# yukara-ikemiya/world-class

Measured on AMD Instinct MI355X. Metric: analysis+synthesis frames/sec (whole node), 48 kHz 5 ms hop, higher is better.
Workload: dtype f64; 1 GPU; 64 synthetic 48 kHz 10 s utterances per GPU (8 distinct, tiled), 5 ms hop, Harvest->CheapTrick->D4C->Synthesis, inputs resident in HBM when the clock starts (`value`; SURVEY.md section 8(d)'s headline with H2D of x and D2H of all outputs inside the clock is `value_with_transfers`); utterances_per_gpu=64, frames_per_gpu=128064, fs=48000, fft_size=2048, parallelism=utterance-sharded x1 (shard.partition), final RCCL all-gather of F0 + checksums

## Files before the change

### world_class_amd/build.py

```python
import hashlib
import os
import re
import subprocess
import sys
from concurrent.futures import ThreadPoolExecutor

HERE = os.path.dirname(os.path.abspath(__file__))
CSRC = os.path.join(HERE, "csrc")
OUT = os.path.join(HERE, "libworldclass_hip.so")
OBJ = os.path.join(HERE, "_obj")
EXTRA = os.environ.get("WC_EXTRA_FLAGS", "").split()
FLAGS = EXTRA + ["--offload-arch=gfx950", "-O3", "-std=c++17", "-fPIC", "-ffp-contract=off", "-munsafe-fp-atomics", "-Wall",
         "-Wno-unused-function", "-Wno-unused-result", "-mllvm", "-simplifycfg-sink-common=false"]
HASH_MARKER = b"WC_SOURCE_HASH="


def sources():
    return sorted(f for f in os.listdir(CSRC) if f.endswith(".hip"))


def headers():
    inc = os.path.join(os.path.dirname(HERE), "include")
    hs = sorted(os.path.join(CSRC, f) for f in os.listdir(CSRC) if f.endswith(".hpp"))
    hs += [os.path.join(inc, f) for f in ("world_class_c.h", "world_class_io.h", "world_class_codec.h", "world_class_stream.h", "world_class_shard.h",
                                          "world_matlabfunctions.hpp", "world_fft.hpp") if os.path.exists(os.path.join(inc, f))]
    return hs


def source_hash():
    h = hashlib.sha256()
    h.update(" ".join(FLAGS).encode())
    for path in [os.path.join(CSRC, f) for f in sources()] + headers():
        h.update(b"\0" + os.path.basename(path).encode() + b"\0")
        with open(path, "rb") as f:
            h.update(f.read())
    return h.hexdigest()


def embedded_hash(path=None):
    path = path or OUT
    if not os.path.exists(path):
        return None
    with open(path, "rb") as f:
        m = re.search(HASH_MARKER + rb"([0-9a-f]{64})", f.read())
    return m.group(1).decode() if m else None


def _stale(out, deps):
    if not os.path.exists(out):
        return True
    t = os.path.getmtime(out)
    return any(os.path.getmtime(d) > t for d in deps)


def build(force=False, verbose=False):
    hipcc = os.environ.get("HIPCC", "/opt/rocm/bin/hipcc")
    want = source_hash()
    if not force and embedded_hash() == want:
        return OUT
    os.makedirs(OBJ, exist_ok=True)
    stamp = os.path.join(OBJ, "flags.txt")
    flags_now = " ".join(FLAGS)
    if not os.path.exists(stamp) or open(stamp).read() != flags_now:
        force = True
    jobs = []
    objs = []
    hs = headers()
    for src in sources():
        s = os.path.join(CSRC, src)
        o = os.path.join(OBJ, src[:-4] + ".o")
        objs.append(o)
        cmd = [hipcc] + FLAGS
        if src == "wc_core.hip":
            cmd += ['-DWC_SOURCE_HASH="%s"' % want]
            jobs.append(cmd + ["-c", s, "-o", o])
        elif force or _stale(o, [s] + hs):
            jobs.append(cmd + ["-c", s, "-o", o])

    def run(cmd):
        if verbose:
            print(" ".join(cmd), flush=True)
        r = subprocess.run(cmd, stdout=subprocess.PIPE, stderr=subprocess.STDOUT, text=True)
        return r.returncode, r.stdout

    with ThreadPoolExecutor(max_workers=4) as ex:
        for rc, out in ex.map(run, jobs):
            if out.strip():
                print(out)
            if rc != 0:
                raise RuntimeError("hipcc failed")
    with open(stamp, "w") as f:
        f.write(flags_now)
    rc, out = run([hipcc, "--offload-arch=gfx950", "-shared", "-fPIC", "-o", OUT] + objs + ["-ldl"])
    if out.strip():
        print(out)
    if rc != 0:
        raise RuntimeError("link failed")
    if embedded_hash() != want:
        raise RuntimeError("built library does not carry the expected source hash")
    return OUT


if __name__ == "__main__":
    print(build(force="--force" in sys.argv, verbose=True))
```

### world_class_amd/csrc/wc_stages.hpp

```cpp
#pragma once
#include <utility>
#include <vector>

#include "wc_internal.hpp"
#include "wc_stretch.hpp"

inline bool fft_size_supported(int fft_size) { return fft_size == 512 || fft_size == 1024 || fft_size == 2048 || fft_size == 4096; }

int hv_enqueue(wc_harvest *h, hipStream_t s, int n_utt, const double *d_x, const int *x_length, double *d_tpos, double *d_f0,
			   bool full, hipEvent_t mid_event, hipEvent_t start_after, int part = 3, hipEvent_t bp_done = nullptr,
			   hipEvent_t tail_after = nullptr);
int hv_overflowed(wc_harvest *h, hipStream_t s, bool *overflow, bool *tie = nullptr, std::vector<int> *tie_utts = nullptr);
std::vector<std::pair<int, int>> hv_runs_of(const std::vector<int> &us);
wc_harvest *hv_exact_twin(wc_harvest *h);
void hv_set_phases(wc_harvest *h, int mask);
int hv_row_width(const wc_harvest *h);
int hv_reserve_rows(wc_harvest *h, long long total_1ms_frames);
double *hv_candidate_rows(wc_harvest *h);
double *hv_score_rows(wc_harvest *h);

int ct_prepare(wc_cheaptrick *c, hipStream_t s, int n_utt, const int *x_length, const double *d_f0, const int *f0_length,
			   const uint64_t *rng_pos, long long *total_out, uint64_t *min_pos_out, uint64_t *max_end_out);
int ct_frames(wc_cheaptrick *c, hipStream_t s, int n_utt, const double *d_x, const double *d_tpos, const double *d_f0,
			  double *d_sp, long long total, hipEvent_t *rows_done);
const unsigned long long *ct_end_positions(const wc_cheaptrick *c);
void ct_set_f0_bound(wc_cheaptrick *c, double f0_bound);
void d4c_set_f0_bound(wc_d4c *d, double f0_bound);

int d4c_enqueue(wc_d4c *d, hipStream_t s, int n_utt, const double *d_x, const int *x_length, const double *d_tpos,
				const double *d_f0, const int *f0_length, int fft_size, double *d_ap, const uint64_t *rng_pos,
				const unsigned long long *d_start);
const unsigned long long *d4c_end_positions(const wc_d4c *d);
uint64_t d4c_draw_bound(const wc_d4c *d, int f0_length);

int syn_prepare(wc_synthesis *sy, hipStream_t s, int n_utt, const double *d_f0, const int *f0_length, const int *out_length,
				double *d_out, const uint64_t *rng_pos, bool full);
int syn_pulses(wc_synthesis *sy, hipStream_t s, const double *d_f0, const double *d_sp, const double *d_ap, double *d_out,
			   const unsigned long long *d_start);
int syn_finish(wc_synthesis *sy, hipStream_t s, uint64_t *rng_pos_out, bool *overflow);

wc::Device *hv_device(const wc_harvest *h);
wc::Device *ct_device(const wc_cheaptrick *c);
wc::Device *d4c_device(const wc_d4c *d);
wc::Device *syn_device(const wc_synthesis *sy);
const double *syn_dc_remover(const wc_synthesis *sy);
int syn_fs(const wc_synthesis *sy);

namespace wc {
struct CodecPlanArgs {
	const int *k;
	const double *s;
	const double2 *w;
};
struct CodecPlan {
	DevBuf k, s, w, kp, sp;
	CodecPlanArgs args() const { return {k.as<int>(), s.as<double>(), w.as<double2>()}; }
	CodecPlanArgs wave_args() const { return {kp.as<int>(), sp.as<double>(), w.as<double2>()}; }
};
int codec_plan(Device *dev, int fs, int fft_size, bool coding, const CodecPlan **out);
int codec_code_sp_launch(Device *dev, hipStream_t st, int fft_size, long long n_frames, int nd, const double *d_sp, double *d_coded,
						 const CodecPlan &pl);
int codec_decode_sp_launch(Device *dev, hipStream_t st, int fft_size, long long n_frames, int nd, const double *d_coded, double *d_sp,
						   const CodecPlan &pl);
int codec_code_ap_launch(hipStream_t st, int fs, int fft_size, long long n_frames, const double *d_ap, double *d_coded);
int codec_decode_ap_launch(hipStream_t st, int fs, int fft_size, long long n_frames, const double *d_coded, double *d_ap);

const char *decode_features_check(int fs, int fft_size, int nd);
int decode_features_enqueue(Device *dev, hipStream_t s, int fs, int fft_size, long long n_frames, int nd, const double *d_coded_sp,
							const double *d_coded_ap, const double *d_spectral_ratio, double *d_sp, double *d_ap);

int modify_frames_enqueue(hipStream_t s, int fs, int fft_size, long long n_frames, double *d_f0, double *d_sp, const double *d_f0_scale,
						  const double *d_spectral_ratio);

const char *retime_check(int fs, int fft_size, int n_utt, const int *in_length, const int *out_length, long long *total_out);
int retime_enqueue(Device *dev, hipStream_t s, int fs, int fft_size, int n_utt, const int *in_length, const double *d_f0_in,
				   const double *d_sp_in, const double *d_ap_in, const int *out_length, const double *d_position, const double *d_f0_scale,
				   const double *d_spectral_ratio, double *d_f0_out, double *d_sp_out, double *d_ap_out, long long total_out);

// ... 6 lines not shown
```

### world_class_amd/csrc/wc_synth_stream.hip

```cpp
#include <algorithm>
#include <cfloat>
#include <climits>
#include <cmath>
#include <cstring>
#include <vector>

#include "wc_stages.hpp"
#include "wc_synthesis.hpp"
#include "../../include/world_class_stream.h"

namespace wc {

struct SsDesc {
	long long win_old, win_new;
	long long in_off;
	int keep_from, keep, n_in;
	int f_base, f_len;
	int n0, n1;
	int cap;
	int has_pend, pend_idx, pend_vuv;
	double pend_shift;
	double run, wrap, vu;
	long long inc_off, slot;
};
// ... 480 lines not shown
		std::memcpy(h + ((char *)d_utt - dm), utt.data(), sizeof(UttDesc) * na);
		std::memcpy(h + ((char *)d_prefix - dm), prefix.data(), sizeof(long long) * (na + 1));
		std::memcpy(h + ((char *)d_capoff - dm), capoff.data(), sizeof(long long) * na);
		std::memcpy(h + ((char *)d_pairs - dm), pairs.data(), sizeof(long long) * 2 * na);
		std::memcpy(h + ((char *)d_first - dm), first.data(), sizeof(int) * na);
		const size_t off = (char *)d_ol - dm, len = ((char *)(d_first + na)) - (char *)d_ol;
		WC_HIP(hipMemcpyAsync(dm + off, h + off, len, hipMemcpyHostToDevice, hs));
		if ((rc = s->h_stage.mark(hs))) return rc;
	}
	double *carry_old = s->carry[par].as<double>(), *carry_new = s->carry[1 - par].as<double>();
	const unsigned tiles = (unsigned)std::max(1, (max_span + SS_TILE - 1) / SS_TILE);
	auto overlap = [&](const double *rows, const double *src, double *dst, const OlDesc *descs) {
		switch (N) {
			case 512: hipLaunchKernelGGL(ss_overlap_kernel<512>, dim3(tiles, na), dim3(SS_T), 0, hs, descs, (const int *)pb.index, rows, src, d_y, dst); break;
			case 1024: hipLaunchKernelGGL(ss_overlap_kernel<1024>, dim3(tiles, na), dim3(SS_T), 0, hs, descs, (const int *)pb.index, rows, src, d_y, dst); break;
			case 2048: hipLaunchKernelGGL(ss_overlap_kernel<2048>, dim3(tiles, na), dim3(SS_T), 0, hs, descs, (const int *)pb.index, rows, src, d_y, dst); break;
			default: hipLaunchKernelGGL(ss_overlap_kernel<4096>, dim3(tiles, na), dim3(SS_T), 0, hs, descs, (const int *)pb.index, rows, src, d_y, dst); break;
		}
	};
	std::vector<OlDesc> ol_expand;
	if (atomic) {
		if ((rc = s->work.reserve(sizeof(double) * (size_t)n * s->wsz))) return rc;
	}
	if (total_p > 0) {
		if (!atomic && (rc = s->resp.reserve(sizeof(double) * (size_t)total_p * N))) return rc;
		SynArgs sa;
		std::memset(&sa, 0, sizeof(sa));
		sa.utts = d_utt; sa.n_utt = na; sa.pulse_prefix = d_prefix; sa.cap_off = d_capoff; sa.first_index = d_first; sa.p = pb;
		sa.f0 = s->wf0[1 - par].as<double>(); sa.sp = s->wsp[1 - par].as<double>(); sa.ap = s->wap[1 - par].as<double>();
		sa.tw = s->dev->twiddle; sa.dc_remover = syn_dc_remover(s->sy);
		sa.out = atomic ? s->work.as<double>() : nullptr;
		sa.resp = atomic ? nullptr : s->resp.as<double>();
		sa.rng_start = nullptr; sa.trace = nullptr; sa.only_pulse = -1; sa.fs = s->fs; sa.frame_period = s->frame_period;
		std::vector<int> owner((size_t)total_p);
		for (int a = 0; a < na; ++a) std::fill(owner.begin() + prefix[a], owner.begin() + prefix[a + 1], a);
		DevBuf &pu = s->owner;
		if ((rc = pu.reserve(sizeof(int) * (size_t)total_p * 2))) return rc;
		WC_HIP(hipMemcpyAsync(pu.p, owner.data(), sizeof(int) * (size_t)total_p, hipMemcpyHostToDevice, hs));
		WC_HIP(hipMemsetAsync(pu.as<int>() + total_p, 0, sizeof(int) * (size_t)total_p, hs));
		WC_HIP(hipStreamSynchronize(hs));
		if (atomic) {
			std::vector<OlDesc> ex(ol);
			for (auto &d : ex) { d.dst_off = d.src_off / s->ccap * s->wsz; d.cut = d.lo; }
			ol_expand = ex;
		}
		uint64_t lo = ~0ull, hi = 0;
		for (int a = 0; a < na; ++a) {
			if (n_syn[a] == 0) continue;
			lo = std::min<uint64_t>(lo, start[a]);
			hi = std::max<uint64_t>(hi, start[a] + (uint64_t)(E[act[a]] - first[a]) + 1);
		}
		if (atomic) {
			if ((rc = s->aux.reserve(sizeof(OlDesc) * na))) return rc;
			WC_HIP(hipMemcpyAsync(s->aux.p, ol_expand.data(), sizeof(OlDesc) * na, hipMemcpyHostToDevice, hs));
			overlap(nullptr, carry_old, s->work.as<double>(), s->aux.as<OlDesc>());
			WC_HIP(hipStreamSynchronize(hs));
		}
		if (hi - lo <= (1ull << 28)) {
			if ((rc = s->dev->ensure_rng(lo, hi))) return rc;
			sa.rng_table = s->dev->rng_table.as<uint32_t>(); sa.rng_base = s->dev->rng_base;
			sa.pulse_utt = pu.as<int>();
			sa.total_pulses = total_p;
			if ((rc = syn_launch_responses(N, sa, hs))) return rc;
		} else {
			for (int a = 0; a < na; ++a) {
				if (n_syn[a] == 0) continue;
// ... 95 lines not shown
```

### world_class_amd/csrc/wc_synthesis.hip

```cpp
#include <cmath>
#include <cstdlib>
#include <cstring>
#include <vector>

#include "wc_device.hpp"
#include "wc_internal.hpp"
#include "wc_frames.hpp"
#include "wc_wavefft.hpp"
#include "wc_hostcopy.hpp"
#include "wc_synthesis.hpp"
#include "wc_stages.hpp"

namespace wc {

constexpr double kSafe = 0.000000000001;

struct TbArgs {
	const UttDesc *utts;
	const double *f0;
	const long long *cap_off;
	const int *cap;
	PulseBuf p;
	int *count;
	int *first_index;
// ... 1024 lines not shown
	wf_r2c_unpack(mr, mi, nyq, tw, lane);
#pragma unroll
	for (int s = 0; s < 16; ++s) {
		const double t = wf_exp_l(mr[s] * (0.5 / N), T);
		double sn, cs;
		wf_sincos(mi[s] * (0.5 / N), sn, cs);
		mr[s] = t * cs;
		mi[s] = t * sn;
	}
	mMr = wf_exp_l(nyq * (0.5 / N), T);
}

#ifndef WC_SYN_WAVE_OCC
#define WC_SYN_WAVE_OCC 2
#endif
#ifndef WC_SYN_ROWS_G
#define WC_SYN_ROWS_G 2
#endif
#ifndef WC_SYN_PARK_NOISE
#define WC_SYN_PARK_NOISE 1
#endif
#ifndef WC_SYN_ROW_PF
#define WC_SYN_ROW_PF 0
#endif
#ifndef WC_SYN_TRACE
#define WC_SYN_TRACE 0
#endif
#if WC_SYN_TRACE
#define SYN_STAMP(i) do { if (lane == 0) a.trace[gp * 16 + (i)] = __builtin_readcyclecounter(); } while (0)
#else
#define SYN_STAMP(i) do { } while (0)
#endif
template <bool ATOMIC>
__global__ __launch_bounds__(64) __attribute__((amdgpu_waves_per_eu(WC_SYN_WAVE_OCC, WC_SYN_WAVE_OCC))) void syn_pulse_wave_kernel(SynArgs a) {
	constexpr int N = 2048, M = 1024;
	__shared__ __attribute__((aligned(16))) double L[kWfLds];
	__shared__ __attribute__((aligned(16))) double T[kWfTabLds];
#if WC_SYN_PARK_NOISE
	__shared__ __attribute__((aligned(16))) double P[1024];
#endif
	const int lane = threadIdx.x;
#ifdef WC_SYN_LDS_PAD
	__shared__ double PAD[WC_SYN_LDS_PAD];
	if (a.fs < 0) PAD[lane] = 0.0;
#endif
	const long long total_p = a.pulse_prefix[a.n_utt];
	if ((long long)blockIdx.x >= 8 * ((total_p + 7) / 8)) return;
	const long long gp = xcd_frame(blockIdx.x, total_p);
	if (gp >= total_p) return;
	if (a.only_pulse >= 0 && gp != a.only_pulse) return;
	const int u = a.pulse_utt[gp];
	wf_tables_to_lds(T, a.tw, lane);
	const UttDesc ud = a.utts[u];
	const long long slot = a.cap_off[u] + (gp - a.pulse_prefix[u]);
	const int pidx = a.p.index[slot];
	const double shift = a.p.shift[slot];
	const int noise_size = a.p.noise_size[slot];
	const double vuv = (double)a.p.vuv[slot];
	const int fs = a.fs, Lf = ud.f_len;
	const double fp = a.frame_period;
	const double t = pidx / (double)fs;

	const int fl = min(Lf - 1, (int)floor(t / fp));
	const int ce = min(Lf - 1, (int)ceil(t / fp));
	const double ipol = uniform_d(t / fp - fl);
	const double *__restrict__ sf = a.sp + (ud.f_off + fl - ud.f_base) * (long long)(M + 1);
	const double *__restrict__ sc = a.sp + (ud.f_off + ce - ud.f_base) * (long long)(M + 1);
	const double *__restrict__ af = a.ap + (ud.f_off + fl - ud.f_base) * (long long)(M + 1);
	const double *__restrict__ ac = a.ap + (ud.f_off + ce - ud.f_base) * (long long)(M + 1);
	const bool same = fl == ce;
	auto blend = [&](double s0, double s1, double a0, double a1, double &env, double &ar) {
		if (same) {
			env = fabs(s0);
			const double s = safe_ap(a0);
			ar = s * s;
		} else {
			env = fma(1.0 - ipol, fabs(s0), ipol * fabs(s1));
			const double s = (1.0 - ipol) * safe_ap(a0) + ipol * safe_ap(a1);
			ar = s * s;
		}
	};
	double ar0;
	{
		double env;
		blend(sf[0], sc[0], af[0], ac[0], env, ar0);
		ar0 = uniform_d(ar0);
	}
#if WC_SYN_ROW_PF > 0
	double pf_s, pf_a;
	{
		const long long r2 = (ud.f_off + min(ce + WC_SYN_ROW_PF, Lf - 1) - ud.f_base) * (long long)(M + 1) + 16 * lane;
		pf_s = a.sp[r2];
		pf_a = a.ap[r2];
	}
#endif
	SYN_STAMP(0);
	SYN_STAMP(1);

	double dc = 0.0;
	const double sq = sqrt((double)noise_size);
#ifdef WC_SYN_RESP_ALIAS
	double *__restrict__ resp = a.resp + (gp & 2047) * (ATOMIC ? M : N);
#else
	double *__restrict__ resp = a.resp + gp * (ATOMIC ? M : N);
#endif
	double *__restrict__ yout = a.out + ud.y_off;
	const int ylen = ud.y_len;
	auto add2 = [&](int o, double v0, double v1) {
		if (o >= 0 && o < ylen) atomicAdd(yout + o, v0);
		if (o + 1 >= 0 && o + 1 < ylen) atomicAdd(yout + o + 1, v1);
	};
	const bool has_periodic = !(vuv <= 0.5 || ar0 > 0.999);
#pragma unroll 1
	for (int part = has_periodic ? 0 : 1; part < 2; ++part) {
		int ln = lane;
		WC_FRESH(ln);
		double wr[16], wi[16];
		double nr[16], ni[16], nsM = 0.0;
		if (part == 1) {
			const unsigned long long rstart = a.rng_start ? a.rng_start[u] : ud.rng_pos;
			const uint32_t *__restrict__ rng = a.rng_table + (rstart + (unsigned long long)(pidx - a.first_index[u]) - a.rng_base);
			double s = 0.0;
			{
				uint32_t raw[32];
#pragma unroll
				for (int q = 0; q < 16; ++q) {
					if ((q & 3) == 0 && q * 128 >= noise_size) break;
					const int i0 = 2 * ln + 128 * q;
					raw[2 * q] = rng[i0 < noise_size ? i0 : 0];
					raw[2 * q + 1] = rng[i0 + 1 < noise_size ? i0 + 1 : 0];
				}
				WF_SCHED_FENCE();
#pragma unroll
				for (int q = 0; q < 16; ++q) {
					nr[q] = ni[q] = 0.0;
					if (q * 128 < ((noise_size + 511) & ~511)) {
						const int i0 = 2 * ln + 128 * q;
						if (i0 < noise_size) nr[q] = raw[2 * q] / 268435456.0 - 6.0;
						if (i0 + 1 < noise_size) ni[q] = raw[2 * q + 1] / 268435456.0 - 6.0;
						s += nr[q] + ni[q];
					}
				}
			}
			s = wave_sum_all(s);
// ... 65 lines not shown
				}
			double sn_, reM;
			wf_sincos(coef * M, sn_, reM);
			yM = mM * reM;
		} else {
#if WC_SYN_PARK_NOISE
			{
				const double *rp = resp;
				asm volatile("" : "+s"(rp));
#pragma unroll
				for (int sI = 0; sI < 16; ++sI) {
					ni[sI] = rp[64 * sI + ln];
					nr[sI] = P[64 * sI + ln];
				}
				WF_SCHED_FENCE();
			}
#endif
#pragma unroll
			for (int sI = 0; sI < 16; ++sI) {
				const double x = wr[sI], y = wi[sI], nx = 0.5 * nr[sI], ny = 0.5 * ni[sI];
				wr[sI] = fma(x, nx, -(y * ny));
				wi[sI] = fma(x, ny, y * nx);
			}
			yM = mM * (0.5 * nsM);
		}
		wf_c2r_pack(wr, wi, yM, a.tw, ln);
		wf_fft1024_dif<-1>(wr, wi, L, a.tw, ln);
		SYN_STAMP(part ? 9 : 4);
		if (part == 0) {
#pragma unroll
			for (int q = 0; q < 8; ++q) {
				dc += wr[q] + wi[q];
				if (ATOMIC) {
					add2(pidx + 1 + 2 * ln + 128 * q, wr[q] * sq / N, wi[q] * sq / N);
				} else {
					*reinterpret_cast<double2 *>(resp + M + 2 * ln + 128 * q) = make_double2(wr[q] * sq, wi[q] * sq);
				}
			}
			dc = wave_sum_all(dc);
			SYN_STAMP(5);
		} else {
			const double dcs = has_periodic ? -dc * sq : 0.0;
			if (ATOMIC) {
#pragma unroll
				for (int q0 = 0; q0 < 8; q0 += 4) {
					double2 dr[4];
#pragma unroll
					for (int q = 0; q < 4; ++q) dr[q] = *reinterpret_cast<const double2 *>(a.dc_remover + 2 * ln + 128 * (q0 + q));
					WF_SCHED_FENCE();
#pragma unroll
					for (int q = 0; q < 4; ++q) {
						const int n = 2 * ln + 128 * (q0 + q);
						add2(pidx + 1 + n, fma(dcs, dr[q].x, wr[q0 + q]) / N, fma(dcs, dr[q].y, wi[q0 + q]) / N);
						add2(pidx + 1 - M + n, fma(dcs, dr[q].x, wr[q0 + q + 8]) / N, fma(dcs, dr[q].y, wi[q0 + q + 8]) / N);
					}
				}
			} else
#pragma unroll
			for (int q0 = 0; q0 < 8; q0 += 4) {
				double2 dr[4], pp[4];
#pragma unroll
				for (int q = 0; q < 4; ++q) {
					dr[q] = *reinterpret_cast<const double2 *>(a.dc_remover + 2 * ln + 128 * (q0 + q));
					pp[q] = has_periodic ? *reinterpret_cast<const double2 *>(resp + M + 2 * ln + 128 * (q0 + q)) : make_double2(0.0, 0.0);
				}
				WF_SCHED_FENCE();
#pragma unroll
				for (int q = 0; q < 4; ++q) {
					const int n = 2 * ln + 128 * (q0 + q);
					const double r0 = fma(dcs, dr[q].x, wr[q0 + q]) + pp[q].x, r1 = fma(dcs, dr[q].y, wi[q0 + q]) + pp[q].y;
					*reinterpret_cast<double2 *>(resp + n + M) = make_double2(r0 / N, r1 / N);
					const double r2 = fma(dcs, dr[q].x, wr[q0 + q + 8]), r3 = fma(dcs, dr[q].y, wi[q0 + q + 8]);
					*reinterpret_cast<double2 *>(resp + n) = make_double2(r2 / N, r3 / N);
				}
			}
			SYN_STAMP(10);
		}
	}
#if WC_SYN_ROW_PF > 0
	asm volatile("" ::"v"(pf_s), "v"(pf_a));
#endif
}

__device__ __forceinline__ void minimum_phase_wave8(double (&mr)[8], double (&mi)[8], double &mMr,
													double *L, const double *T, const double2 *__restrict__ tw, int lane) {
	constexpr int N = 1024, M = 512;
	WC_FRESH(lane);
	int jg[2];
#pragma unroll
	for (int g = 0; g < 2; ++g) jg[g] = wf8_bin(lane, g, 0);
	wf_fence();
#pragma unroll
	for (int q = 0; q < 4; ++q) {
		const double2 v = *reinterpret_cast<const double2 *>(&L[2 * lane + 128 * q]);
		mr[q] = v.x;
		mi[q] = v.y;
	}
#pragma unroll
	for (int q = 4; q < 8; ++q) {
		mr[q] = L[1024 - 2 * lane - 128 * q];
		mi[q] = L[1023 - 2 * lane - 128 * q];
	}
	wf_fence();
	wf8_fft512_dit<+1>(mr, mi, L, tw, lane);
	double nyq;
	wf8_r2c_unpack_re(mr, mi, nyq, tw, lane);
#pragma unroll
	for (int g = 0; g < 2; ++g)
#pragma unroll
		for (int q = 0; q < 4; ++q) L[jg[g] + 128 * q] = (g == 0 && q == 0 && lane == 0) ? 0.5 * mr[0] : mr[4 * g + q];
	if (lane == 0) L[M] = 0.5 * nyq;
	wf_fence();
#pragma unroll
	for (int q = 0; q < 4; ++q) {
// ... 269 lines not shown
				v[b][m] = (on && j >= 0 && j < N) ? rows[(long long)ii * N + j] : 0.0;
			}
		}
#pragma unroll
		for (int b = 0; b < PB; ++b)
#pragma unroll
			for (int m = 0; m < OA_K; ++m) acc[m] += v[b][m];
	}
	double *__restrict__ out = a.out + ud.y_off;
#pragma unroll
	for (int m = 0; m < OA_K; ++m) {
		const int o = o0 + m * OA_T;
		if (o < ud.y_len) out[o] = acc[m];
	}
}

}

using namespace wc;

struct wc_synthesis {
	int fs, fft_size;
	double frame_period;
	Device *dev;
	wc_synthesis *twin = nullptr;
	hipStream_t s_twin = nullptr;
	hipEvent_t e_twin = nullptr;
	bool is_twin = false;
	DevBuf dc_remover, utts, meta, pulses, incs, phase, phase_seg, tile_cnt, resp, pulse_utt, d_f0, d_sp, d_ap, d_out;
	bool pulses_by_utterance;
	bool wave;
	bool rows = false;
	bool wave_atomic = false;
	size_t rows_budget = 0;
	bool phase_single;
	bool serial_timebase;
	HostBuf h_stage, h_rows;
	DevBuf dec_sp, dec_ap;
	DevBuf rt_f0, rt_sp, rt_ap;
	long long total_out = 0, cap_total = 0;
	int n_utt = 0, max_out = 0;
};

template <int N>
static void launch_pulses(const SynArgs &a, hipStream_t s) {
	constexpr int TP = (N >= 2048) ? 256 : (N / 8 < 64 ? 64 : N / 8);
	hipLaunchKernelGGL((syn_pulse_kernel<N, TP>), dim3((unsigned)(8 * ((a.total_pulses + 7) / 8))), dim3(TP), 0, s, a);
}

int wc::syn_launch_responses(int fft_size, const SynArgs &a, hipStream_t s) {
	switch (fft_size) {
		case 512: launch_pulses<512>(a, s); break;
		case 1024: {
			const long long per = (a.total_pulses + 7) / 8;
			hipLaunchKernelGGL(syn_pulse_wave8_kernel, dim3((unsigned)(8 * ((per + kSyn8Waves - 1) / kSyn8Waves))), dim3(64 * kSyn8Waves), 0, s, a);
			break;
		}
		case 2048: hipLaunchKernelGGL(syn_pulse_wave_kernel<false>, dim3((unsigned)(8 * ((a.total_pulses + 7) / 8))), dim3(64), 0, s, a); break;
		case 4096: launch_pulses<4096>(a, s); break;
		default: return fail(WC_ERR_UNSUPPORTED, "synthesis: fft_size must be 512, 1024, 2048 or 4096");
	}
	WC_HIP(hipGetLastError());
	return WC_OK;
}

__global__ void syn_prefix_kernel(int n_utt, const int *__restrict__ count, const int *__restrict__ cap,
								  const int *__restrict__ first_index, const int *__restrict__ last_index,
								  const UttDesc *__restrict__ utts, const unsigned long long *__restrict__ d_start,
								  long long *__restrict__ prefix, unsigned long long *__restrict__ end_pos, int *__restrict__ overflow) {
	if (threadIdx.x != 0) return;
	long long run = 0;
	int ovf = 0;
	for (int u = 0; u < n_utt; ++u) {
		prefix[u] = run;
		if (count[u] > cap[u]) ovf = 1;
		run += min(count[u], cap[u]);
		const unsigned long long st = d_start ? d_start[u] : utts[u].rng_pos;
		end_pos[u] = st + (unsigned long long)(last_index[u] - first_index[u]);
	}
	prefix[n_utt] = run;
	*overflow = ovf;
}

int syn_prepare(wc_synthesis *sy, hipStream_t s, int n_utt, const double *d_f0, const int *f0_length, const int *out_length,
				double *d_out, const uint64_t *rng_pos, bool full) {
	Device *dev = sy->dev;
	std::vector<UttDesc> utts(n_utt);
	long long fo = 0, yo = 0;
	int max_out = 0;
	for (int u = 0; u < n_utt; ++u) {
		if (f0_length[u] < 2) return fail(WC_ERR_INVALID, "synthesis: f0_length must be at least 2 (reference src/synthesis.cpp:241-242)");
		if (out_length[u] < 0) return fail(WC_ERR_INVALID, "synthesis: negative out_length");
		UttDesc &t = utts[u];
		t.x_off = 0; t.f_off = fo; t.y_off = yo; t.x_len = 0; t.f_len = f0_length[u]; t.y_len = out_length[u]; t.f_base = 0;
		t.rng_pos = rng_pos ? rng_pos[u] : 0ull;
		fo += f0_length[u];
		yo += out_length[u];
		max_out = std::max(max_out, out_length[u]);
	}
	const long long total_out = yo;
	sy->total_out = total_out;
	sy->n_utt = n_utt;
	sy->max_out = max_out;
	sy->cap_total = 0;
	if (total_out == 0) return WC_OK;
	int rc;
	const size_t meta_bytes = sizeof(long long) * (4 * (size_t)n_utt + 1) + sizeof(int) * (4 * (size_t)n_utt + 1);
	if ((rc = sy->utts.reserve(sizeof(UttDesc) * n_utt))) return rc;
	if ((rc = sy->meta.reserve(meta_bytes))) return rc;
	if ((rc = sy->h_stage.reserve(sizeof(UttDesc) * n_utt + meta_bytes))) return rc;
	char *hs = static_cast<char *>(sy->h_stage.p);
	std::memcpy(hs, utts.data(), sizeof(UttDesc) * n_utt);
	long long *h_cap_off = reinterpret_cast<long long *>(hs + sizeof(UttDesc) * n_utt);
	long long *h_inc_off = h_cap_off + 2 * n_utt + 1;
	int *h_cap = reinterpret_cast<int *>(h_cap_off + 4 * n_utt + 1);
	char *dm = static_cast<char *>(sy->meta.p);
	long long *d_cap_off = reinterpret_cast<long long *>(dm);
	long long *d_prefix = d_cap_off + n_utt;
	long long *d_inc_off = d_prefix + n_utt + 1;
	unsigned long long *d_end = reinterpret_cast<unsigned long long *>(d_inc_off + n_utt);
	int *d_cap = reinterpret_cast<int *>(d_end + n_utt);
	int *d_count = d_cap + n_utt;
	int *d_first = d_count + n_utt;
	int *d_last = d_first + n_utt;
	long long inc_total = 0, co = 0;
	for (int u = 0; u < n_utt; ++u) {
		h_inc_off[u] = inc_total;
		inc_total += ((long long)out_length[u] + 63) / 64 * 64 + 64;
		const long long soft = (long long)out_length[u] * 960 / sy->fs + 16;
		const int cap = (full || soft > out_length[u]) ? out_length[u] + 1 : (int)soft;
		h_cap_off[u] = co;
		h_cap[u] = cap;
		co += cap;
	}
	sy->cap_total = co;
	sy->rows = sy->wave && (sy->fft_size == 2048 || sy->fft_size == 1024) &&
			   (double)co * sy->fft_size * sizeof(double) <= (double)sy->rows_budget;
	if (!sy->rows || (sy->wave_atomic && sy->fft_size == 2048)) WC_HIP(hipMemsetAsync(d_out, 0, sizeof(double) * total_out, s));
	if ((rc = sy->incs.reserve(sizeof(double) * inc_total))) return rc;
	if (!sy->serial_timebase && (rc = sy->phase.reserve(sizeof(double) * inc_total))) return rc;
// ... 49 lines not shown
							   (const double *)sy->phase.as<double>(), sy->tile_cnt.as<int>(), max_tiles);
			hipLaunchKernelGGL(syn_pulse_tiles_kernel<1>, dim3(max_tiles, n_utt), dim3(TB_T), 0, s, ta, (const double *)sy->incs.as<double>(),
							   (const double *)sy->phase.as<double>(), sy->tile_cnt.as<int>(), max_tiles);
		}
	}
	hipLaunchKernelGGL(syn_noise_size_kernel, dim3(8, n_utt), dim3(256), 0, s, d_cap_off, d_count, d_cap, pb, d_first, d_last);
	WC_HIP(hipGetLastError());
	return dev->time_end("synthesis_timebase", s);
}

int syn_pulses(wc_synthesis *sy, hipStream_t s, const double *d_f0, const double *d_sp, const double *d_ap, double *d_out,
			   const unsigned long long *d_start) {
	Device *dev = sy->dev;
	if (sy->total_out == 0 || sy->cap_total == 0) return WC_OK;
	const int n_utt = sy->n_utt;
	int rc;
	char *dm = static_cast<char *>(sy->meta.p);
	long long *d_cap_off = reinterpret_cast<long long *>(dm);
	long long *d_prefix = d_cap_off + n_utt;
	long long *d_inc_off = d_prefix + n_utt + 1;
	unsigned long long *d_end = reinterpret_cast<unsigned long long *>(d_inc_off + n_utt);
	int *d_cap = reinterpret_cast<int *>(d_end + n_utt);
	int *d_count = d_cap + n_utt;
	int *d_first = d_count + n_utt;
	int *d_last = d_first + n_utt;
	int *d_ovf = d_last + n_utt;
	const long long co = sy->cap_total;
	PulseBuf pb;
	pb.shift = sy->pulses.as<double>();
	pb.index = reinterpret_cast<int *>(pb.shift + co);
	pb.noise_size = pb.index + co;
	pb.vuv = pb.noise_size + co;
	hipLaunchKernelGGL(syn_prefix_kernel, dim3(1), dim3(64), 0, s, n_utt, d_count, d_cap, d_first, d_last, sy->utts.as<UttDesc>(),
					   d_start, d_prefix, d_end, d_ovf);
	SynArgs a;
	a.utts = sy->utts.as<UttDesc>(); a.n_utt = n_utt; a.pulse_prefix = d_prefix; a.cap_off = d_cap_off;
	a.first_index = d_first; a.p = pb; a.f0 = d_f0; a.sp = d_sp; a.ap = d_ap;
	a.rng_table = dev->rng_table.as<uint32_t>(); a.rng_base = dev->rng_base; a.tw = dev->twiddle;
	a.dc_remover = sy->dc_remover.as<double>(); a.out = d_out; a.total_pulses = co; a.fs = sy->fs;
	a.frame_period = sy->frame_period; a.rng_start = d_start;
#ifdef WC_DEBUG_HOOKS
	{
		const char *dbg = getenv("WC_DEBUG_ONLY_PULSE");
		a.only_pulse = dbg ? atoll(dbg) : -1;
	}
#else
	a.only_pulse = -1;
#endif
	a.trace = nullptr;
	a.resp = nullptr;
	a.pulse_utt = nullptr;
	if (sy->rows) {
		const bool atomic_rows = sy->wave_atomic && sy->fft_size == 2048;
		if ((rc = sy->resp.reserve(sizeof(double) * (size_t)(atomic_rows ? sy->fft_size / 2 : sy->fft_size) * (size_t)co))) return rc;
		a.resp = sy->resp.as<double>();
		if ((rc = sy->pulse_utt.reserve(sizeof(int) * (size_t)co))) return rc;
		a.pulse_utt = sy->pulse_utt.as<int>();
		hipLaunchKernelGGL(syn_pulse_utt_kernel, dim3(n_utt), dim3(256), 0, s, (const long long *)d_prefix, sy->pulse_utt.as<int>());
	}
#if WC_SYN_TRACE
	static DevBuf tracebuf;
	if (tracebuf.reserve(sizeof(unsigned long long) * 16 * (size_t)co)) return WC_ERR_DEVICE;
	(void)hipMemsetAsync(tracebuf.p, 0, sizeof(unsigned long long) * 16 * (size_t)co, s);
	a.trace = tracebuf.as<unsigned long long>();
#endif
	if ((rc = dev->time_begin("synthesis_pulses", s))) return rc;
	switch (sy->fft_size) {
		case 512: launch_pulses<512>(a, s); break;
		case 1024:
			if (sy->rows) {
				const long long per = (a.total_pulses + 7) / 8;
				hipLaunchKernelGGL(syn_pulse_wave8_kernel, dim3((unsigned)(8 * ((per + kSyn8Waves - 1) / kSyn8Waves))), dim3(64 * kSyn8Waves), 0, s, a);
				hipLaunchKernelGGL(syn_overlap_add_kernel<1024>, dim3((unsigned)((sy->max_out + OA_TILE - 1) / OA_TILE), n_utt), dim3(OA_T), 0, s, a);
			} else {
				launch_pulses<1024>(a, s);
			}
			break;
		case 2048:
			if (sy->rows) {
				if (sy->wave_atomic) {
					hipLaunchKernelGGL(syn_pulse_wave_kernel<true>, dim3((unsigned)(8 * ((a.total_pulses + 7) / 8))), dim3(64), 0, s, a);
				} else {
					hipLaunchKernelGGL(syn_pulse_wave_kernel<false>, dim3((unsigned)(8 * ((a.total_pulses + 7) / 8))), dim3(64), 0, s, a);
					hipLaunchKernelGGL(syn_overlap_add_kernel<2048>, dim3((unsigned)((sy->max_out + OA_TILE - 1) / OA_TILE), n_utt), dim3(OA_T), 0, s, a);
				}
			} else {
				launch_pulses<2048>(a, s);
			}
			break;
		case 4096: launch_pulses<4096>(a, s); break;
		default: return fail(WC_ERR_UNSUPPORTED, "synthesis: fft_size must be 512, 1024, 2048 or 4096");
	}
	WC_HIP(hipGetLastError());
#if WC_SYN_TRACE
	if (const char *path = getenv("WC_SYN_TRACE_FILE")) {
		std::vector<unsigned long long> h((size_t)16 * co);
		WC_HIP(hipStreamSynchronize(s));
		WC_HIP(hipMemcpy(h.data(), a.trace, sizeof(unsigned long long) * h.size(), hipMemcpyDeviceToHost));
		if (FILE *f = fopen(path, "wb")) { fwrite(h.data(), 8, h.size(), f); fclose(f); }
	}
#endif
	return dev->time_end("synthesis_pulses", s);
}

int syn_finish(wc_synthesis *sy, hipStream_t s, uint64_t *rng_pos_out, bool *overflow) {
	*overflow = false;
	if (sy->total_out == 0 || sy->cap_total == 0) return WC_OK;
	const int n_utt = sy->n_utt;
	char *dm = static_cast<char *>(sy->meta.p);
	long long *d_cap_off = reinterpret_cast<long long *>(dm);
	unsigned long long *d_end = reinterpret_cast<unsigned long long *>(d_cap_off + 3 * n_utt + 1);
	int *d_ovf = reinterpret_cast<int *>(d_end + n_utt) + 4 * n_utt;
	int ovf = 0;
	std::vector<uint64_t> ends(n_utt);
	WC_HIP(hipMemcpyAsync(&ovf, d_ovf, sizeof(int), hipMemcpyDeviceToHost, s));
	if (rng_pos_out) WC_HIP(hipMemcpyAsync(ends.data(), d_end, sizeof(uint64_t) * n_utt, hipMemcpyDeviceToHost, s));
// ... 50 lines not shown
			dev->time_tag = 1;
			WC_HIP(hipEventRecord(sy->e_twin, s));
			WC_HIP(hipStreamWaitEvent(sB, sy->e_twin, 0));
			if (runB && (rc = syn_pulses(syB, sB, d_f0 + foA, d_sp + foA * bins, d_ap + foA * bins, d_out + yoA, nullptr))) return bail(rc);
			dev->time_tag = -1;
			bool oA = false, oB = false;
			if (runA && (rc = syn_finish(sy, s, endA, &oA))) return bail(rc);
			if (runB && (rc = syn_finish(syB, sB, endB, &oB))) return bail(rc);
			if (!runA) WC_HIP(hipStreamSynchronize(s));
			if (!runB) WC_HIP(hipStreamSynchronize(sB));
			if (!oA && !oB) {
				if (rng_pos) std::copy(rng_end.begin(), rng_end.end(), rng_pos);
				return WC_OK;
			}
			runA = oA; runB = oB;
			fullA = fullA || oA;
			fullB = fullB || oB;
		}
		return fail(WC_ERR_DEVICE, "synthesis: pulse buffer overflow");
	}
	for (int attempt = 0; attempt < 2; ++attempt) {
		if ((rc = syn_prepare(sy, s, n_utt, d_f0, f0_length, out_length, d_out, rng_pos, attempt == 1))) return rc;
		if ((rc = syn_pulses(sy, s, d_f0, d_sp, d_ap, d_out, nullptr))) return rc;
		bool overflow = false;
		if ((rc = syn_finish(sy, s, rng_pos, &overflow))) return rc;
		if (!overflow) return WC_OK;
	}
	return fail(WC_ERR_DEVICE, "synthesis: pulse buffer overflow");
}

wc::Device *syn_device(const wc_synthesis *sy) { return sy->dev; }
int syn_fs(const wc_synthesis *sy) { return sy->fs; }
const double *syn_dc_remover(const wc_synthesis *sy) { return sy->dc_remover.as<double>(); }

extern "C" {

wc_synthesis *wc_synthesis_create(int fs, int fft_size, double frame_period_ms) {
	if (fs <= 0 || frame_period_ms <= 0) { set_error("synthesis: fs and frame_period must be positive"); return nullptr; }
	if (!fft_size_supported(fft_size)) {
		set_error("synthesis: fft_size must be 512, 1024, 2048 or 4096");
		return nullptr;
	}
	Device *dev = current_device();
	if (!dev) return nullptr;
	wc_synthesis *s = new wc_synthesis();
	s->fs = fs;
	s->fft_size = fft_size;
	s->frame_period = frame_period_ms / 1000.;
	{
		const char *tb = getenv("WC_SYN_TIMEBASE");
		s->serial_timebase = tb && std::string(tb) == "serial";
		const char *ph = getenv("WC_SYN_PHASE");
		s->phase_single = ph && std::string(ph) == "single";
		const char *pu = getenv("WC_SYN_PULSES");
		s->pulses_by_utterance = pu && std::string(pu) == "utterance";
		const char *impl = getenv("WC_SYN_IMPL");
		s->wave = !(impl && std::string(impl) == "block");
		const char *ola = getenv("WC_SYN_OLA");
		s->wave_atomic = ola && std::string(ola) == "atomic";
		size_t free_b = 0, total_b = 0;
		if (hipMemGetInfo(&free_b, &total_b) != hipSuccess) total_b = (size_t)64 << 30;
		s->rows_budget = total_b / 8;
		if (const char *mb = getenv("WC_SYN_ROWS_BUDGET_MB")) s->rows_budget = (size_t)atoll(mb) << 20;
	}
	s->dev = dev;
	std::vector<double> d(fft_size);
	const double cv = 2.0 * 3.1415926535897932384 / (1.0 + fft_size);
	for (int i = 0; i < fft_size / 2; ++i) d[i] = 0.5 - 0.5 * std::cos(cv * (i + 1.0));
	double dc = 0.0;
	for (int i = 0; i < fft_size / 2; ++i) dc += d[i];
	dc *= 2;
	for (int i = 0; i < fft_size / 2; ++i) { d[i] /= dc; d[fft_size - i - 1] = d[i]; }
	if (s->dc_remover.reserve(sizeof(double) * fft_size) ||
		hipMemcpy(s->dc_remover.p, d.data(), sizeof(double) * fft_size, hipMemcpyHostToDevice) != hipSuccess) {
		set_error("synthesis: table upload failed");
		delete s;
		return nullptr;
	}
	dev->handle_born();
	return s;
}
void wc_synthesis_destroy(wc_synthesis *s) {
	if (!s) return;
	s->dev->quiesce();
	s->dev->handle_gone();
	if (s->twin) wc_synthesis_destroy(s->twin);
	if (s->s_twin) (void)hipStreamDestroy(s->s_twin);
	if (s->e_twin) (void)hipEventDestroy(s->e_twin);
	s->dc_remover.release(); s->utts.release(); s->meta.release(); s->pulses.release(); s->incs.release(); s->phase.release(); s->tile_cnt.release(); s->phase_seg.release(); s->resp.release(); s->pulse_utt.release();
	s->d_f0.release(); s->d_sp.release(); s->d_ap.release(); s->d_out.release(); s->h_stage.release(); s->h_rows.release();
	s->dec_sp.release(); s->dec_ap.release();
	s->rt_f0.release(); s->rt_sp.release(); s->rt_ap.release();
	delete s;
}

int wc_synthesis_get_fft_size(const wc_synthesis *s) { return s ? s->fft_size : WC_ERR_INVALID; }
// ... 107 lines not shown
```

### world_class_amd/csrc/wc_synthesis.hpp

```cpp
#pragma once
#include <cstdint>

#include "wc_device.hpp"
#include "wc_internal.hpp"

namespace wc {

struct PulseBuf {
	int *index;
	double *shift;
	int *noise_size;
	int *vuv;
};

struct Coarse {
	const double *f0;
	int L;
	double lowest_f0, fp;
	int base = 0;
	__device__ __forceinline__ double cf_in(int j) const {
		double v = f0[j - base];
		return (v < lowest_f0) ? 0.0 : v;
	}
	__device__ __forceinline__ double cv_in(int j) const { return (cf_in(j) == 0.0) ? 0.0 : 1.0; }
// ... 91 lines not shown
		"s_waitcnt lgkmcnt(0)\n\t"
		"v_add_f64 %[m], %[m], |s[56:57]|\n\t s_lshl_b64 exec, exec, 1\n\t"
		"v_add_f64 %[m], %[m], |s[58:59]|\n\t s_lshl_b64 exec, exec, 1\n\t"
		"v_add_f64 %[m], %[m], |s[60:61]|\n\t s_lshl_b64 exec, exec, 1\n\t"
		"v_add_f64 %[m], %[m], |s[62:63]|\n\t s_lshl_b64 exec, exec, 1\n\t"
		"v_add_f64 %[m], %[m], |s[64:65]|\n\t s_lshl_b64 exec, exec, 1\n\t"
		"v_add_f64 %[m], %[m], |s[66:67]|\n\t s_lshl_b64 exec, exec, 1\n\t"
		"v_add_f64 %[m], %[m], |s[68:69]|\n\t s_lshl_b64 exec, exec, 1\n\t"
		"v_add_f64 %[m], %[m], |s[70:71]|\n\t s_lshl_b64 exec, exec, 1\n\t"
		"s_mov_b64 exec, %[sv]\n\t"
		: [m] "+v"(mine), [sv] "=&s"(save)
		: [p] "s"(p)
		: "scc", "memory", "s40", "s41", "s42", "s43", "s44", "s45", "s46", "s47", "s48", "s49", "s50", "s51", "s52", "s53",
		  "s54", "s55", "s56", "s57", "s58", "s59", "s60", "s61", "s62", "s63", "s64", "s65", "s66", "s67", "s68", "s69", "s70",
		  "s71");
}

struct SynArgs {
	const UttDesc *utts;
	int n_utt;
	const long long *pulse_prefix;
	const long long *cap_off;
	const int *first_index;
	PulseBuf p;
	const double *f0, *sp, *ap;
	const uint32_t *rng_table;
	unsigned long long rng_base;
	const double2 *tw;
	const double *dc_remover;
	double *out;
	const int *pulse_utt;
	double *resp;
	long long total_pulses;
	const unsigned long long *rng_start;
	unsigned long long *trace;
	long long only_pulse;
	int fs;
	double frame_period;
};

int syn_launch_responses(int fft_size, const SynArgs &a, hipStream_t s);

}
```

Measured before the change: 5.144 million frames/s.

## Make synthesis pulse-wave kernel persistent with atomic ticket work distribution

```diff
diff --git a/world_class_amd/build.py b/world_class_amd/build.py
--- a/world_class_amd/build.py
+++ b/world_class_amd/build.py
@@ -12,6 +12,7 @@
 EXTRA = os.environ.get("WC_EXTRA_FLAGS", "").split()
 FLAGS = EXTRA + ["--offload-arch=gfx950", "-O3", "-std=c++17", "-fPIC", "-ffp-contract=off", "-munsafe-fp-atomics", "-Wall",
          "-Wno-unused-function", "-Wno-unused-result", "-mllvm", "-simplifycfg-sink-common=false"]
+FILE_FLAGS = {"wc_synthesis.hip": ["-mllvm", "-disable-machine-licm"]}
 HASH_MARKER = b"WC_SOURCE_HASH="
 
 
@@ -30,6 +31,7 @@
 def source_hash():
     h = hashlib.sha256()
     h.update(" ".join(FLAGS).encode())
+    h.update(repr(sorted(FILE_FLAGS.items())).encode())
     for path in [os.path.join(CSRC, f) for f in sources()] + headers():
         h.update(b"\0" + os.path.basename(path).encode() + b"\0")
         with open(path, "rb") as f:
@@ -60,7 +62,7 @@
         return OUT
     os.makedirs(OBJ, exist_ok=True)
     stamp = os.path.join(OBJ, "flags.txt")
-    flags_now = " ".join(FLAGS)
+    flags_now = " ".join(FLAGS) + " " + repr(sorted(FILE_FLAGS.items()))
     if not os.path.exists(stamp) or open(stamp).read() != flags_now:
         force = True
     jobs = []
@@ -70,7 +72,7 @@
         s = os.path.join(CSRC, src)
         o = os.path.join(OBJ, src[:-4] + ".o")
         objs.append(o)
-        cmd = [hipcc] + FLAGS
+        cmd = [hipcc] + FLAGS + FILE_FLAGS.get(src, [])
         if src == "wc_core.hip":
             cmd += ['-DWC_SOURCE_HASH="%s"' % want]
             jobs.append(cmd + ["-c", s, "-o", o])
diff --git a/world_class_amd/csrc/wc_stages.hpp b/world_class_amd/csrc/wc_stages.hpp
--- a/world_class_amd/csrc/wc_stages.hpp
+++ b/world_class_amd/csrc/wc_stages.hpp
@@ -44,6 +44,7 @@
 wc::Device *d4c_device(const wc_d4c *d);
 wc::Device *syn_device(const wc_synthesis *sy);
 const double *syn_dc_remover(const wc_synthesis *sy);
+int syn_grid_cap(const wc_synthesis *sy);
 int syn_fs(const wc_synthesis *sy);
 
 namespace wc {
diff --git a/world_class_amd/csrc/wc_synth_stream.hip b/world_class_amd/csrc/wc_synth_stream.hip
--- a/world_class_amd/csrc/wc_synth_stream.hip
+++ b/world_class_amd/csrc/wc_synth_stream.hip
@@ -536,6 +536,7 @@
 		sa.out = atomic ? s->work.as<double>() : nullptr;
 		sa.resp = atomic ? nullptr : s->resp.as<double>();
 		sa.rng_start = nullptr; sa.trace = nullptr; sa.only_pulse = -1; sa.fs = s->fs; sa.frame_period = s->frame_period;
+		sa.grid_cap = syn_grid_cap(s->sy); sa.ticket = nullptr;
 		std::vector<int> owner((size_t)total_p);
 		for (int a = 0; a < na; ++a) std::fill(owner.begin() + prefix[a], owner.begin() + prefix[a + 1], a);
 		DevBuf &pu = s->owner;
diff --git a/world_class_amd/csrc/wc_synthesis.hip b/world_class_amd/csrc/wc_synthesis.hip
--- a/world_class_amd/csrc/wc_synthesis.hip
+++ b/world_class_amd/csrc/wc_synthesis.hip
@@ -1080,25 +1080,12 @@
 #define SYN_STAMP(i) do { } while (0)
 #endif
 template <bool ATOMIC>
-__global__ __launch_bounds__(64) __attribute__((amdgpu_waves_per_eu(WC_SYN_WAVE_OCC, WC_SYN_WAVE_OCC))) void syn_pulse_wave_kernel(SynArgs a) {
+__device__ __forceinline__ void syn_pulse_wave(const SynArgs &a, const long long gp, double *__restrict__ L, const double *__restrict__ T,
+											   double *__restrict__ P, int lane) {
 	constexpr int N = 2048, M = 1024;
-	__shared__ __attribute__((aligned(16))) double L[kWfLds];
-	__shared__ __attribute__((aligned(16))) double T[kWfTabLds];
-#if WC_SYN_PARK_NOISE
-	__shared__ __attribute__((aligned(16))) double P[1024];
-#endif
-	const int lane = threadIdx.x;
-#ifdef WC_SYN_LDS_PAD
-	__shared__ double PAD[WC_SYN_LDS_PAD];
-	if (a.fs < 0) PAD[lane] = 0.0;
-#endif
-	const long long total_p = a.pulse_prefix[a.n_utt];
-	if ((long long)blockIdx.x >= 8 * ((total_p + 7) / 8)) return;
-	const long long gp = xcd_frame(blockIdx.x, total_p);
-	if (gp >= total_p) return;
+	WC_FRESH(lane);
 	if (a.only_pulse >= 0 && gp != a.only_pulse) return;
 	const int u = a.pulse_utt[gp];
-	wf_tables_to_lds(T, a.tw, lane);
 	const UttDesc ud = a.utts[u];
 	const long long slot = a.cap_off[u] + (gp - a.pulse_prefix[u]);
 	const int pidx = a.p.index[slot];
@@ -1158,6 +1145,7 @@
 		if (o >= 0 && o < ylen) atomicAdd(yout + o, v0);
 		if (o + 1 >= 0 && o + 1 < ylen) atomicAdd(yout + o + 1, v1);
 	};
+	const int pidx_s = ATOMIC ? __builtin_amdgcn_readfirstlane(pidx) : pidx;
 	const bool has_periodic = !(vuv <= 0.5 || ar0 > 0.999);
 #pragma unroll 1
 	for (int part = has_periodic ? 0 : 1; part < 2; ++part) {
@@ -1289,7 +1277,7 @@
 			for (int q = 0; q < 8; ++q) {
 				dc += wr[q] + wi[q];
 				if (ATOMIC) {
-					add2(pidx + 1 + 2 * ln + 128 * q, wr[q] * sq / N, wi[q] * sq / N);
+					add2(pidx_s + 1 + 2 * ln + 128 * q, wr[q] * sq / N, wi[q] * sq / N);
 				} else {
 					*reinterpret_cast<double2 *>(resp + M + 2 * ln + 128 * q) = make_double2(wr[q] * sq, wi[q] * sq);
 				}
@@ -1308,8 +1296,8 @@
 #pragma unroll
 					for (int q = 0; q < 4; ++q) {
 						const int n = 2 * ln + 128 * (q0 + q);
-						add2(pidx + 1 + n, fma(dcs, dr[q].x, wr[q0 + q]) / N, fma(dcs, dr[q].y, wi[q0 + q]) / N);
-						add2(pidx + 1 - M + n, fma(dcs, dr[q].x, wr[q0 + q + 8]) / N, fma(dcs, dr[q].y, wi[q0 + q + 8]) / N);
+						add2(pidx_s + 1 + n, fma(dcs, dr[q].x, wr[q0 + q]) / N, fma(dcs, dr[q].y, wi[q0 + q]) / N);
+						add2(pidx_s + 1 - M + n, fma(dcs, dr[q].x, wr[q0 + q + 8]) / N, fma(dcs, dr[q].y, wi[q0 + q + 8]) / N);
 					}
 				}
 			} else
@@ -1337,6 +1325,40 @@
 #if WC_SYN_ROW_PF > 0
 	asm volatile("" ::"v"(pf_s), "v"(pf_a));
 #endif
+}
+
+template <bool ATOMIC>
+__global__ __launch_bounds__(64) __attribute__((amdgpu_waves_per_eu(WC_SYN_WAVE_OCC, WC_SYN_WAVE_OCC))) void syn_pulse_wave_kernel(SynArgs a) {
+	__shared__ __attribute__((aligned(16))) double L[kWfLds];
+	__shared__ __attribute__((aligned(16))) double T[kWfTabLds];
+#if WC_SYN_PARK_NOISE
+	__shared__ __attribute__((aligned(16))) double P[1024];
+#else
+	double *P = nullptr;
+#endif
+	const int lane = threadIdx.x;
+#ifdef WC_SYN_LDS_PAD
+	__shared__ double PAD[WC_SYN_LDS_PAD];
+	if (a.fs < 0) PAD[lane] = 0.0;
+#endif
+	const long long total_p = a.pulse_prefix[a.n_utt];
+	const long long per = (total_p + 7) / 8, first = (long long)(blockIdx.x & 7) * per;
+	const long long step = gridDim.x >> 3;
+	long long i = blockIdx.x >> 3;
+	if (i >= per || first + i >= total_p) return;
+	wf_tables_to_lds(T, a.tw, lane);
+#pragma unroll 1
+	for (;;) {
+		if (a.ticket) {
+			unsigned t = 0;
+			if (lane == 0) t = atomicAdd(a.ticket + (blockIdx.x & 7), 1u);
+			i = __builtin_amdgcn_readfirstlane(t);
+		}
+		if (i >= per || first + i >= total_p) break;
+		syn_pulse_wave<ATOMIC>(a, first + i, L, T, P, lane);
+		wf_fence();
+		i += step;
+	}
 }
 
 __device__ __forceinline__ void minimum_phase_wave8(double (&mr)[8], double (&mi)[8], double &mMr,
@@ -1672,6 +1694,8 @@
 	bool wave;
 	bool rows = false;
 	bool wave_atomic = false;
+	int grid_cap = 0;
+	bool ticket = true;
 	size_t rows_budget = 0;
 	bool phase_single;
 	bool serial_timebase;
@@ -1688,6 +1712,28 @@
 	hipLaunchKernelGGL((syn_pulse_kernel<N, TP>), dim3((unsigned)(8 * ((a.total_pulses + 7) / 8))), dim3(TP), 0, s, a);
 }
 
+#ifndef WC_SYN_GRID_K
+#define WC_SYN_GRID_K 1
+#endif
+static int syn_wave_resident(bool atomic) {
+	int per_cu = 0, dev_id = 0;
+	hipDeviceProp_t prop;
+	hipError_t e = atomic ? hipOccupancyMaxActiveBlocksPerMultiprocessor(&per_cu, syn_pulse_wave_kernel<true>, 64, 0)
+						  : hipOccupancyMaxActiveBlocksPerMultiprocessor(&per_cu, syn_pulse_wave_kernel<false>, 64, 0);
+	if (e != hipSuccess || hipGetDevice(&dev_id) != hipSuccess || hipGetDeviceProperties(&prop, dev_id) != hipSuccess || per_cu < 1) {
+		(void)hipGetLastError();
+		return 0;
+	}
+	return per_cu * prop.multiProcessorCount * WC_SYN_GRID_K;
+}
+
+template <bool ATOMIC>
+static void launch_pulse_wave(const SynArgs &a, hipStream_t s) {
+	long long grid = 8 * ((a.total_pulses + 7) / 8);
+	if (a.grid_cap > 0) grid = std::min<long long>(grid, 8 * (((long long)a.grid_cap + 7) / 8));
+	hipLaunchKernelGGL(syn_pulse_wave_kernel<ATOMIC>, dim3((unsigned)grid), dim3(64), 0, s, a);
+}
+
 int wc::syn_launch_responses(int fft_size, const SynArgs &a, hipStream_t s) {
 	switch (fft_size) {
 		case 512: launch_pulses<512>(a, s); break;
@@ -1696,7 +1742,7 @@
 			hipLaunchKernelGGL(syn_pulse_wave8_kernel, dim3((unsigned)(8 * ((per + kSyn8Waves - 1) / kSyn8Waves))), dim3(64 * kSyn8Waves), 0, s, a);
 			break;
 		}
-		case 2048: hipLaunchKernelGGL(syn_pulse_wave_kernel<false>, dim3((unsigned)(8 * ((a.total_pulses + 7) / 8))), dim3(64), 0, s, a); break;
+		case 2048: launch_pulse_wave<false>(a, s); break;
 		case 4096: launch_pulses<4096>(a, s); break;
 		default: return fail(WC_ERR_UNSUPPORTED, "synthesis: fft_size must be 512, 1024, 2048 or 4096");
 	}
@@ -1707,7 +1753,9 @@
 __global__ void syn_prefix_kernel(int n_utt, const int *__restrict__ count, const int *__restrict__ cap,
 								  const int *__restrict__ first_index, const int *__restrict__ last_index,
 								  const UttDesc *__restrict__ utts, const unsigned long long *__restrict__ d_start,
-								  long long *__restrict__ prefix, unsigned long long *__restrict__ end_pos, int *__restrict__ overflow) {
+								  long long *__restrict__ prefix, unsigned long long *__restrict__ end_pos, int *__restrict__ overflow,
+								  unsigned int *__restrict__ ticket) {
+	if (threadIdx.x < 8) ticket[threadIdx.x] = 0u;
 	if (threadIdx.x != 0) return;
 	long long run = 0;
 	int ovf = 0;
@@ -1745,7 +1793,7 @@
 	sy->cap_total = 0;
 	if (total_out == 0) return WC_OK;
 	int rc;
-	const size_t meta_bytes = sizeof(long long) * (4 * (size_t)n_utt + 1) + sizeof(int) * (4 * (size_t)n_utt + 1);
+	const size_t meta_bytes = sizeof(long long) * (4 * (size_t)n_utt + 1) + sizeof(int) * (4 * (size_t)n_utt + 1 + 8);
 	if ((rc = sy->utts.reserve(sizeof(UttDesc) * n_utt))) return rc;
 	if ((rc = sy->meta.reserve(meta_bytes))) return rc;
 	if ((rc = sy->h_stage.reserve(sizeof(UttDesc) * n_utt + meta_bytes))) return rc;
@@ -1861,13 +1909,15 @@
 	pb.noise_size = pb.index + co;
 	pb.vuv = pb.noise_size + co;
 	hipLaunchKernelGGL(syn_prefix_kernel, dim3(1), dim3(64), 0, s, n_utt, d_count, d_cap, d_first, d_last, sy->utts.as<UttDesc>(),
-					   d_start, d_prefix, d_end, d_ovf);
+					   d_start, d_prefix, d_end, d_ovf, reinterpret_cast<unsigned int *>(d_ovf + 1));
 	SynArgs a;
 	a.utts = sy->utts.as<UttDesc>(); a.n_utt = n_utt; a.pulse_prefix = d_prefix; a.cap_off = d_cap_off;
 	a.first_index = d_first; a.p = pb; a.f0 = d_f0; a.sp = d_sp; a.ap = d_ap;
 	a.rng_table = dev->rng_table.as<uint32_t>(); a.rng_base = dev->rng_base; a.tw = dev->twiddle;
 	a.dc_remover = sy->dc_remover.as<double>(); a.out = d_out; a.total_pulses = co; a.fs = sy->fs;
 	a.frame_period = sy->frame_period; a.rng_start = d_start;
+	a.grid_cap = sy->grid_cap;
+	a.ticket = (sy->grid_cap > 0 && sy->ticket) ? reinterpret_cast<unsigned int *>(d_ovf + 1) : nullptr;
 #ifdef WC_DEBUG_HOOKS
 	{
 		const char *dbg = getenv("WC_DEBUG_ONLY_PULSE");
@@ -1908,9 +1958,9 @@
 		case 2048:
 			if (sy->rows) {
 				if (sy->wave_atomic) {
-					hipLaunchKernelGGL(syn_pulse_wave_kernel<true>, dim3((unsigned)(8 * ((a.total_pulses + 7) / 8))), dim3(64), 0, s, a);
+					launch_pulse_wave<true>(a, s);
 				} else {
-					hipLaunchKernelGGL(syn_pulse_wave_kernel<false>, dim3((unsigned)(8 * ((a.total_pulses + 7) / 8))), dim3(64), 0, s, a);
+					launch_pulse_wave<false>(a, s);
 					hipLaunchKernelGGL(syn_overlap_add_kernel<2048>, dim3((unsigned)((sy->max_out + OA_TILE - 1) / OA_TILE), n_utt), dim3(OA_T), 0, s, a);
 				}
 			} else {
@@ -2027,6 +2077,7 @@
 wc::Device *syn_device(const wc_synthesis *sy) { return sy->dev; }
 int syn_fs(const wc_synthesis *sy) { return sy->fs; }
 const double *syn_dc_remover(const wc_synthesis *sy) { return sy->dc_remover.as<double>(); }
+int syn_grid_cap(const wc_synthesis *sy) { return sy->grid_cap; }
 
 extern "C" {
 
@@ -2057,6 +2108,10 @@
 		if (hipMemGetInfo(&free_b, &total_b) != hipSuccess) total_b = (size_t)64 << 30;
 		s->rows_budget = total_b / 8;
 		if (const char *mb = getenv("WC_SYN_ROWS_BUDGET_MB")) s->rows_budget = (size_t)atoll(mb) << 20;
+		const char *gr = getenv("WC_SYN_GRID");
+		const bool padded = gr && std::string(gr) == "padded";
+		s->grid_cap = (fft_size == 2048 && s->wave && !padded) ? syn_wave_resident(s->wave_atomic) : 0;
+		s->ticket = !(gr && std::string(gr) == "stride");
 	}
 	s->dev = dev;
 	std::vector<double> d(fft_size);
diff --git a/world_class_amd/csrc/wc_synthesis.hpp b/world_class_amd/csrc/wc_synthesis.hpp
--- a/world_class_amd/csrc/wc_synthesis.hpp
+++ b/world_class_amd/csrc/wc_synthesis.hpp
@@ -147,6 +147,8 @@
 	const int *pulse_utt;
 	double *resp;
 	long long total_pulses;
+	int grid_cap;
+	unsigned int *ticket;
 	const unsigned long long *rng_start;
 	unsigned long long *trace;
 	long long only_pulse;
```

Result: no change. 5.174 million frames/s, median of 6 (+0.6%).
